# Brown-LEMS/Edge_Based_Visual_Odometry

Measured on AMD Instinct MI355X. Metric: stereo pairs/sec (TOED+NCC match) on KITTI 1241×376; achieved HBM GB/s, higher is better.
Workload: dtype f64; 1 GPU; configs[1]: single KITTI-shaped stereo pair 1241x376 (generator S2, scene 7+rank, 12 px disparity), TOED both images (fp64, no FMA, bit-exact) + epipolar/disparity/orientation candidate search + NCC, resident in HBM, replayed; toed_mode=hybrid, edges_left=126184, edges_right=126340, candidate_pairs=581657, ncc_matches=472947, sims_stored=False, pairs_in_flight_per_gpu=6, streams_per_gpu=4, pairs_submitted_as_hipgraph=2331, toed_strict_fallbacks=0, parallelism=1 independent sequence(s), one per GPU, no collective

## Files before the change

edge_based_visual_odometry_amd/csrc/match_kernels.hip:

```cpp
#include <atomic>
#include <cstdlib>

#include "ebvo_cand.h"
#include "ebvo_internal.h"
#include "ebvo_math.h"

namespace
{

constexpr int BATCH = 64;
constexpr int TILE = 64;
constexpr int STAGE = 64;
struct DevPairs
{
    int64_t host;
    const int32_t *row_ptr;
    DevN nL;
    int64_t cap;
};
__device__ inline int64_t devpairs(const DevPairs &d)
{
    const int64_t n = d.row_ptr ? (int64_t)d.row_ptr[devn(d.nL)] : d.host;
    return n < d.cap ? n : d.cap;
}

__device__ inline void lines_body(const double *__restrict__ F, const ebvo_edge *__restrict__ e, int n, double *__restrict__ lines,
                                  int vb, int vg)
{
    for (int k = vb * blockDim.x + threadIdx.x; k < n; k += vg * blockDim.x)
    {
        const double x = e[k].x, y = e[k].y;
#pragma unroll
        for (int r = 0; r < 3; ++r)
            lines[(size_t)k * 3 + r] = (F[r * 3 + 0] * x + F[r * 3 + 1] * y) + F[r * 3 + 2];
    }
}

__global__ void lines_kernel(const double *__restrict__ F, const ebvo_edge *__restrict__ e, DevN nd,
                             double *__restrict__ lines)
{
    lines_body(F, e, devn(nd), lines, blockIdx.x, gridDim.x);
}

__global__ __launch_bounds__(256) void boxes_kernel(const ebvo_edge *__restrict__ R, DevN nRd, Box *__restrict__ cb,
                                                    Box *__restrict__ gb, int32_t *__restrict__ tile_flag, int ntiles)
{
    boxes_body(R, devn(nRd), cb, gb, tile_flag, ntiles, blockIdx.x, gridDim.x);
}

__device__ inline Box region_box(const LeftCtx &l, double D, double band, int mask)
{
    const double inf = __builtin_inf();
    Box r;
    r.x0 = -inf; r.x1 = inf; r.y0 = -inf; r.y1 = inf;
    if (mask & EBVO_STAGE_DISPARITY)
    {
        r.x0 = l.lx - D; r.x1 = l.lx + D; r.y0 = l.ly - D; r.y1 = l.ly + D;
    }
    if ((mask & EBVO_STAGE_EPIPOLAR) && (mask & EBVO_STAGE_DISPARITY) && l.ah == l.ah && l.bh == l.bh && l.ch == l.ch)
    {
        const double m = 1e-9;
        if (fabs(l.bh) > m)
        {
            const double ya = -(l.ah * r.x0 + l.ch) / l.bh, yb = -(l.ah * r.x1 + l.ch) / l.bh;
            const double e = band / fabs(l.bh) + BOX_SLACK;
            r.y0 = fmax(r.y0, fmin(ya, yb) - e);
            r.y1 = fmin(r.y1, fmax(ya, yb) + e);
        }
        if (fabs(l.ah) > m)
        {
            const double xa = -(l.bh * r.y0 + l.ch) / l.ah, xb = -(l.bh * r.y1 + l.ch) / l.ah;
            const double e = band / fabs(l.ah) + BOX_SLACK;
            r.x0 = fmax(r.x0, fmin(xa, xb) - e);
            r.x1 = fmin(r.x1, fmax(xa, xb) + e);
        }
    }
    return r;
}

template <bool FILL, bool COPY = FILL>
__global__ __launch_bounds__(256) void candidates_kernel(const ebvo_edge *__restrict__ L,
                                                         const ebvo_edge *__restrict__ R,
                                                         const double *__restrict__ lines,
                                                         const Box *__restrict__ cb, const Box *__restrict__ gb,
                                                         CandParams P, int32_t *__restrict__ cnt,
                                                         const int32_t *__restrict__ row_ptr,
                                                         int32_t *__restrict__ col_idx,
                                                         unsigned long long *__restrict__ total_part)
{
    __shared__ double s_x[BATCH * CHUNK], s_y[BATCH * CHUNK], s_th[BATCH * CHUNK];
    __shared__ Box s_box[BATCH];
    __shared__ LeftCtx s_left[TILE];
    __shared__ int s_round[256];
    __shared__ int s_groups[256];
    __shared__ int s_wcnt[4];
    __shared__ double s_red[4];
    __shared__ unsigned long long s_tot[4];

    const int tid = threadIdx.x, lane = tid & 63, wid = tid >> 6;
    constexpr int LPE = CHUNK, GPB = 256 / LPE, ROUNDS = TILE / GPB;
    constexpr unsigned long long GMASK = (1ull << LPE) - 1ull;
    static_assert(TILE % GPB == 0 && BATCH % LPE == 0 && BATCH <= 64, "tile rounds / marked-chunk mask");
    const int gid = tid / LPE, e = tid % LPE, gshift = lane & ~(LPE - 1);
    const int nL = devn(P.nL), nR = devn(P.nR);
    const int nchunks = (nR + CHUNK - 1) / CHUNK, ngroups = (nchunks + GROUP - 1) / GROUP;
    const double d2 = P.max_disp * P.max_disp;
    const double D = P.max_disp + BOX_SLACK, band = P.epi_thr + BOX_SLACK;
    const double inf = __builtin_inf();
    unsigned long long blk_total = 0;

    auto compact = [&](bool sel, int value, int *list) -> int {
        const unsigned long long m = __ballot(sel);
        if (lane == 0)
            s_wcnt[wid] = __popcll(m);
        __syncthreads();
        int pre = 0, tot = 0;
#pragma unroll
        for (int k = 0; k < 4; ++k)
        {
            if (k < wid) pre += s_wcnt[k];
            tot += s_wcnt[k];
        }
        if (sel)
            list[pre + __popcll(m & ((1ull << lane) - 1ull))] = value;
        __syncthreads();
        return tot;
    };

    if (!FILL && blockIdx.x == 0 && tid == 0)
        cnt[nL] = 0;
    if (FILL && COPY)
    {
        const int e16 = tid & 15;
        const int rows = (gridDim.x * 256) >> 4;
        for (int i = (blockIdx.x * 256 + tid) >> 4; i < nL; i += rows)
        {
            const int64_t o = row_ptr[i];
            const int n = row_ptr[i + 1] - row_ptr[i];
            if (n > STAGE)
                continue;
            for (int k = e16; k < n; k += 16)
                if (o + k < P.cap)
                    col_idx[o + k] = P.stage[(size_t)i * STAGE + k];
        }
    }
    for (int tile = blockIdx.x; tile * TILE < nL; tile += gridDim.x)
    {
        if (FILL && !P.tile_flag[tile])
            continue;
        if (wid == 0)
        {
            const int i = tile * TILE + lane;
            const bool live = i < nL;
            const int il = live ? i : 0;
            const LeftCtx l = left_ctx_make(L[il].x, L[il].y, L[il].theta, lines[(size_t)il * 3], lines[(size_t)il * 3 + 1],
                                            lines[(size_t)il * 3 + 2], P.epi_thr, d2);
            Box rb = region_box(l, D, band, P.mask);
            if (!live) { rb.x0 = inf; rb.x1 = -inf; rb.y0 = inf; rb.y1 = -inf; }
            s_left[lane] = l;
            const double a0 = wave_min(rb.x0), a1 = wave_max(rb.x1), b0 = wave_min(rb.y0), b1 = wave_max(rb.y1);
            if (lane == 0) { s_red[0] = a0; s_red[1] = a1; s_red[2] = b0; s_red[3] = b1; }
        }
        __syncthreads();
        Box U;
        U.x0 = s_red[0]; U.x1 = s_red[1]; U.y0 = s_red[2]; U.y1 = s_red[3];
        auto meets_union = [&](const Box &bx) {
            return !(bx.x0 > U.x1 || bx.x1 < U.x0 || bx.y0 > U.y1 || bx.y1 < U.y0);
        };

        int n[ROUNDS];
        int64_t o[ROUNDS];
#pragma unroll
        for (int r = 0; r < ROUNDS; ++r)
        {
            n[r] = 0;
            o[r] = 0;
        }
        if (FILL)
        {
#pragma unroll
            for (int r = 0; r < ROUNDS; ++r)
            {
                const int i = tile * TILE + r * GPB + gid;
                o[r] = (int64_t)row_ptr[i < nL ? i : 0];
            }
        }
        for (int g0 = 0; g0 < ngroups; g0 += 256)
        {
            const int g = g0 + tid;
            const int ngsel = compact(g < ngroups && meets_union(gb[g < ngroups ? g : 0]), g, s_groups);
            for (int q = 0; q < ngsel; q += 4)
            {
                const int gq = q + (tid >> 6);
                const int c = (gq < ngsel) ? s_groups[gq] * GROUP + (tid & 63) : nchunks;
                const int nsel = compact(c < nchunks && meets_union(cb[c < nchunks ? c : 0]), c, s_round);
                for (int b0 = 0; b0 < nsel; b0 += BATCH)
                {
                    const int mb = min(BATCH, nsel - b0);
                    for (int idx = tid; idx < mb * CHUNK; idx += 256)
                    {
                        const int k = s_round[b0 + idx / CHUNK] * CHUNK + (idx % CHUNK);
                        double x = __builtin_nan(""), y = x, th = x;
                        if (k < nR)
                        {
                            x = R[k].x; y = R[k].y; th = R[k].theta;
                        }
                        s_x[idx] = x; s_y[idx] = y; s_th[idx] = th;
                    }
                    if (tid < mb)
                        s_box[tid] = cb[s_round[b0 + tid]];
                    __syncthreads();
#pragma unroll
                    for (int r = 0; r < ROUNDS; ++r)
                    {
                        const int li = r * GPB + gid;
                        const int i = tile * TILE + li;
                        const bool live = i < nL;
                        const LeftCtx l = s_left[li];
                        unsigned long long pm = 0;
#pragma unroll
                        for (int k = 0; k < BATCH / LPE; ++k)
                        {
                            const int j = k * LPE + e;
                            const bool may = live && j < mb &&
                                             box_may_match(s_box[j < mb ? j : 0], l.lx, l.ly, l.ah, l.bh, l.ch, D, band,
                                                           P.mask);
                            const unsigned long long bal = __ballot(may);
                            pm |= ((bal >> gshift) & GMASK) << (LPE * k);
                        }
                        while (__any(pm != 0))
                        {
                            const bool act = pm != 0;
                            const int j = act ? __ffsll((long long)pm) - 1 : 0;
                            pm &= pm - 1;
                            const int idx = j * CHUNK + e;
                            const bool ok = act && pair_passes(l, s_x[idx], s_y[idx], s_th[idx], P);
                            const unsigned hits = (unsigned)((__ballot(ok) >> gshift) & GMASK);
                            if (ok)
                            {
                                const int rank = __popc(hits & ((1u << e) - 1u));
                                const int k = s_round[b0 + j] * CHUNK + e;
                                if (FILL)
                                {
                                    if (o[r] + rank < P.cap)
                                        col_idx[o[r] + rank] = k;
                                }
                                else if (n[r] + rank < STAGE)
                                    P.stage[(size_t)i * STAGE + n[r] + rank] = k;
                            }
                            const int nh = __popc(hits);
                            n[r] += nh;
                            o[r] += nh;
                        }
                    }
                    __syncthreads();
                }
            }
        }
        if (!FILL)
        {
            unsigned long long tsum = 0;
#pragma unroll
            for (int r = 0; r < ROUNDS; ++r)
            {
                const int i = tile * TILE + r * GPB + gid;
                if (e == 0 && i < nL)
                {
                    cnt[i] = n[r];
                    if (n[r] > STAGE)
                        P.tile_flag[tile] = 1;
                    tsum += (unsigned long long)n[r];
                }
            }
            for (int d = 32; d > 0; d >>= 1)
                tsum += __shfl_down(tsum, d);
            if (lane == 0)
                s_tot[wid] = tsum;
            __syncthreads();
            if (tid == 0)
            {
                const unsigned long long t = s_tot[0] + s_tot[1] + s_tot[2] + s_tot[3];
                blk_total += t;
                P.tile_tot[tile] = (int32_t)(uint32_t)t;
            }
        }
        __syncthreads();
    }
    if (!FILL && tid == 0)
        total_part[blockIdx.x] = blk_total;
}

__global__ void total_sum_kernel(const unsigned long long *__restrict__ part, int n, unsigned long long *__restrict__ total)
{
    unsigned long long v = 0;
    for (int k = threadIdx.x; k < n; k += 64)
        v += part[k];
    for (int d = 32; d > 0; d >>= 1)
        v += __shfl_down(v, d);
    if (threadIdx.x == 0)
        *total = v;
}

__global__ void candidates_copy_kernel(const int32_t *__restrict__ row_ptr, const int32_t *__restrict__ stage, DevN nLd,
                                       int64_t cap, int32_t *__restrict__ col_idx)
{
    const int nL = devn(nLd);
    const int e = threadIdx.x & 15;
    const int rows = (gridDim.x * blockDim.x) >> 4;
    for (int i = (blockIdx.x * blockDim.x + threadIdx.x) >> 4; i < nL; i += rows)
    {
        const int64_t o = row_ptr[i];
        const int n = row_ptr[i + 1] - row_ptr[i];
        if (n > STAGE)
            continue;
        for (int k = e; k < n; k += 16)
            if (o + k < cap)
                col_idx[o + k] = stage[(size_t)i * STAGE + k];
    }
}

struct ClearList
{
    int32_t *p[EBVO_CLEAR_MAX];
    int n[EBVO_CLEAR_MAX];
};
__global__ void clear_kernel(ClearList C)
{
    int32_t *__restrict__ p = C.p[blockIdx.y];
    const int n = C.n[blockIdx.y];
    for (int k = blockIdx.x * blockDim.x + threadIdx.x; k < n; k += gridDim.x * blockDim.x)
        p[k] = 0;
}

constexpr int SCAN_ITEMS = 16;
constexpr int SCAN_BLOCK = 256;
constexpr int SCAN_TILE = SCAN_ITEMS * SCAN_BLOCK;
constexpr int SCAN_BATCH = 4;
constexpr int SCAN_DIRECT_TILES = 16;

struct ScanBatch
{
    const int32_t *in[SCAN_BATCH];
    int32_t *out[SCAN_BATCH];
    DevN n[SCAN_BATCH];
    int n_add;
    int32_t *total[SCAN_BATCH];
    int32_t *sums;
    int tiles;
    int direct;
};

__device__ inline int32_t block_sum_256(int32_t v, int32_t *wsum)
{
    for (int d = 32; d > 0; d >>= 1)
        v += __shfl_down(v, d);
    if ((threadIdx.x & 63) == 0)
        wsum[threadIdx.x >> 6] = v;
    __syncthreads();
    return wsum[0] + wsum[1] + wsum[2] + wsum[3];
}

__global__ __launch_bounds__(SCAN_BLOCK) void scan_reduce_kernel(ScanBatch S)
{
    __shared__ int32_t wsum[SCAN_BLOCK / 64];
    const int a = blockIdx.y;
    const int n_in = devn(S.n[a]), n = n_in + S.n_add;
    const int base = blockIdx.x * SCAN_TILE;
    if (base >= n)
        return;
    const int32_t *__restrict__ in = S.in[a];
    int32_t v = 0;
#pragma unroll
    for (int t = 0; t < SCAN_ITEMS; ++t)
    {
        const int k = base + t * SCAN_BLOCK + threadIdx.x;
        v += (k < n_in) ? in[k] : 0;
    }
    const int32_t tot = block_sum_256(v, wsum);
    if (threadIdx.x == 0)
        S.sums[(size_t)a * S.tiles + blockIdx.x] = tot;
}

__global__ __launch_bounds__(SCAN_BLOCK) void scan_apply_kernel(ScanBatch S)
{
    __shared__ int32_t wsum[SCAN_BLOCK / 64], wpre[SCAN_BLOCK / 64];
    const int a = blockIdx.y;
    const int n_in = devn(S.n[a]), n = n_in + S.n_add;
    const int base = blockIdx.x * SCAN_TILE + threadIdx.x * SCAN_ITEMS;
    if (blockIdx.x * SCAN_TILE >= n)
        return;
    const int32_t *__restrict__ in = S.in[a];
    int32_t *__restrict__ out = S.out[a];
    int32_t o = 0;
    if (S.direct)
    {
        const int before = min((int)blockIdx.x * SCAN_TILE, n_in);
        if ((reinterpret_cast<uintptr_t>(in) & 15) == 0)
        {
            const int4 *p4 = reinterpret_cast<const int4 *>(in);
            for (int k = threadIdx.x; k < (before >> 2); k += SCAN_BLOCK)
            {
                const int4 q = p4[k];
                o += (q.x + q.y) + (q.z + q.w);
            }
            for (int k = (before & ~3) + threadIdx.x; k < before; k += SCAN_BLOCK)
                o += in[k];
        }
        else
            for (int k = threadIdx.x; k < before; k += SCAN_BLOCK)
                o += in[k];
    }
    else
        for (int k = threadIdx.x; k < (int)blockIdx.x; k += SCAN_BLOCK)
            o += S.sums[(size_t)a * S.tiles + k];
    const int32_t tile_off = block_sum_256(o, wpre);
    int32_t v[SCAN_ITEMS];
    int32_t s = 0;
    if (base + SCAN_ITEMS <= n_in && (reinterpret_cast<uintptr_t>(in + base) & 15) == 0)
    {
        const int4 *p = reinterpret_cast<const int4 *>(in + base);
#pragma unroll
        for (int t = 0; t < SCAN_ITEMS / 4; ++t)
        {
            const int4 q = p[t];
            v[4 * t] = q.x; v[4 * t + 1] = q.y; v[4 * t + 2] = q.z; v[4 * t + 3] = q.w;
        }
    }
    else
    {
#pragma unroll
        for (int t = 0; t < SCAN_ITEMS; ++t)
            v[t] = (base + t < n_in) ? in[base + t] : 0;
    }
#pragma unroll
    for (int t = 0; t < SCAN_ITEMS; ++t)
        s += v[t];
    const int lane = threadIdx.x & 63, wid = threadIdx.x >> 6;
    int32_t incl = s;
    for (int d = 1; d < 64; d <<= 1)
    {
        const int32_t t = __shfl_up(incl, d);
        if (lane >= d)
            incl += t;
    }
    if (lane == 63)
        wsum[wid] = incl;
    __syncthreads();
    int32_t pre = 0;
#pragma unroll
    for (int k = 0; k < SCAN_BLOCK / 64; ++k)
        if (k < wid)
            pre += wsum[k];
    int32_t run = tile_off + pre + incl - s;
#pragma unroll
    for (int t = 0; t < SCAN_ITEMS; ++t)
    {
        if (base + t < n)
            out[base + t] = run;
        if (S.n_add == 1 && base + t == n_in && S.total[a])
            *S.total[a] = run;
        run += v[t];
    }
}

__global__ void gather_edges_kernel(const ebvo_edge *__restrict__ R, const int32_t *__restrict__ idx, int64_t n,
                                    ebvo_edge *__restrict__ out)
{
    const int64_t k = (int64_t)blockIdx.x * blockDim.x + threadIdx.x;
    if (k < n)
        out[k] = R[idx[k]];
}

__device__ inline double bilinear_nan(const uint8_t *__restrict__ img, int rows, int cols, int pitch, double x,
                                      double y)
{
    const double x1 = floor(x), x2 = ceil(x);
    const double yc = ceil(y), yf = floor(y);
    const bool inside = (x1 >= 0) && (yf >= 0) && (x2 < cols) && (yc < rows);
    const int c1 = inside ? (int)x1 : 0;
    const int r1 = inside ? (int)yc * pitch : 0, r2 = inside ? (int)yf * pitch : 0;
    unsigned short p1, p2;
    __builtin_memcpy(&p1, img + r1 + c1, 2);
    __builtin_memcpy(&p2, img + r2 + c1, 2);
    const double I11 = (double)(p1 & 0xff);
    const double I21 = (double)(p1 >> 8);
    const double I12 = (double)(p2 & 0xff);
    const double I22 = (double)(p2 >> 8);
    const double wxa = x2 - x;
    const double wxb = x - x1;
    const double wya = -(yf - y);
    const double wyb = -(y - yc);
    const double f1 = wxa * I11 + wxb * I21;
    const double f2 = wxa * I12 + wxb * I22;
    const double v = wya * f1 + wyb * f2;
    const bool ok = inside && (x2 != x1) && (yf != yc);
    return ok ? v : __builtin_nan("");
}

template <int CTRL>
__device__ inline double dpp_f64(double v)
{
    const int lo = __double2loint(v), hi = __double2hiint(v);
    const int plo = __builtin_amdgcn_update_dpp(0, lo, CTRL, 0xf, 0xf, true);
    const int phi = __builtin_amdgcn_update_dpp(0, hi, CTRL, 0xf, 0xf, true);
    return __hiloint2double(phi, plo);
}

__device__ inline double butterfly8(double s)
{
    s += dpp_f64<0xB1>(s);
    s += dpp_f64<0x4E>(s);
    s += dpp_f64<0x141>(s);
    return s;
}

struct PatchBatch
{
    const uint8_t *img[2];
    const ebvo_edge *edges[2];
    DevN n[2];
    double2 *sc[2];
    float *raw[2], *norm[2];
    uint8_t *flag[2];
};

__device__ inline void sincos_body(const ebvo_edge *__restrict__ e, int n, double2 *__restrict__ sc, int vb, int vg)
{
    for (int k = vb * blockDim.x + threadIdx.x; k < n; k += vg * blockDim.x)
    {
        double sn, cs;
        ebvo_sincos(e[k].theta, &sn, &cs);
        double2 v;
// ... 1666 lines not shown
```

Measured before the change: 3524 stereo pairs/s.

## Use precomputed region-box overlap test for flat epipolar bands in candidate search

For each left edge, the region box and a flag saying whether its epipolar band is nearly axis-aligned are now stored in shared memory. For flagged edges, the per-chunk box_may_match test is replaced by a cheaper four-compare overlap ballot against that stored box. Other edges use an inlined box test built on raw v_min/v_max f64 instructions. The change also stages boxes for all batch slots and masks the result with a staged-bit mask, and sets launch_bounds to 4 blocks per CU. The overlap test on flat regions is looser than the epipolar test, so more chunks may reach pair_passes, and the inline-asm min/max drops NaN handling.

```diff
diff --git a/edge_based_visual_odometry_amd/csrc/match_kernels.hip b/edge_based_visual_odometry_amd/csrc/match_kernels.hip
--- a/edge_based_visual_odometry_amd/csrc/match_kernels.hip
+++ b/edge_based_visual_odometry_amd/csrc/match_kernels.hip
@@ -48,6 +48,31 @@
     boxes_body(R, devn(nRd), cb, gb, tile_flag, ntiles, blockIdx.x, gridDim.x);
 }
 
+__device__ inline double fmin_q(double a, double b)
+{
+    double r;
+    asm("v_min_f64 %0, %1, %2" : "=v"(r) : "v"(a), "v"(b));
+    return r;
+}
+__device__ inline double fmax_q(double a, double b)
+{
+    double r;
+    asm("v_max_f64 %0, %1, %2" : "=v"(r) : "v"(a), "v"(b));
+    return r;
+}
+__device__ inline double wave_min_q(double v)
+{
+    for (int d = 32; d > 0; d >>= 1)
+        v = fmin_q(v, __shfl_xor(v, d));
+    return v;
+}
+__device__ inline double wave_max_q(double v)
+{
+    for (int d = 32; d > 0; d >>= 1)
+        v = fmax_q(v, __shfl_xor(v, d));
+    return v;
+}
+
 __device__ inline Box region_box(const LeftCtx &l, double D, double band, int mask)
 {
     const double inf = __builtin_inf();
@@ -64,22 +89,59 @@
         {
             const double ya = -(l.ah * r.x0 + l.ch) / l.bh, yb = -(l.ah * r.x1 + l.ch) / l.bh;
             const double e = band / fabs(l.bh) + BOX_SLACK;
-            r.y0 = fmax(r.y0, fmin(ya, yb) - e);
-            r.y1 = fmin(r.y1, fmax(ya, yb) + e);
+            r.y0 = fmax_q(r.y0, fmin_q(ya, yb) - e);
+            r.y1 = fmin_q(r.y1, fmax_q(ya, yb) + e);
         }
         if (fabs(l.ah) > m)
         {
             const double xa = -(l.bh * r.y0 + l.ch) / l.ah, xb = -(l.bh * r.y1 + l.ch) / l.ah;
             const double e = band / fabs(l.ah) + BOX_SLACK;
-            r.x0 = fmax(r.x0, fmin(xa, xb) - e);
-            r.x1 = fmin(r.x1, fmax(xa, xb) + e);
+            r.x0 = fmax_q(r.x0, fmin_q(xa, xb) - e);
+            r.x1 = fmin_q(r.x1, fmax_q(xa, xb) + e);
         }
     }
     return r;
 }
 
+__device__ inline bool box_may_match_q(const Box &bx, double xl, double yl, double ah, double bh, double ch, double D,
+                                       double band, int mask)
+{
+    double x0 = bx.x0, x1 = bx.x1, y0 = bx.y0, y1 = bx.y1;
+    bool out = false;
+    if (mask & EBVO_STAGE_DISPARITY)
+    {
+        x0 = fmax_q(x0, xl - D);
+        x1 = fmin_q(x1, xl + D);
+        y0 = fmax_q(y0, yl - D);
+        y1 = fmin_q(y1, yl + D);
+        out = x0 > x1 || y0 > y1;
+    }
+    if (mask & EBVO_STAGE_EPIPOLAR)
+    {
+        const double gx0 = ah * x0, gx1 = ah * x1, gy0 = bh * y0, gy1 = bh * y1;
+        const double gmin = fmin_q(gx0, gx1) + fmin_q(gy0, gy1) + ch;
+        const double gmax = fmax_q(gx0, gx1) + fmax_q(gy0, gy1) + ch;
+        out = out || gmin > band || gmax < -band;
+    }
+    return !out;
+}
+
+__device__ inline unsigned long long region_ballot(const Box bx, const Box r)
+{
+    constexpr int UGE = 11, ULE = 13;
+    return __builtin_amdgcn_fcmp(bx.x0, r.x1, ULE) & __builtin_amdgcn_fcmp(bx.x1, r.x0, UGE) &
+           __builtin_amdgcn_fcmp(bx.y0, r.y1, ULE) & __builtin_amdgcn_fcmp(bx.y1, r.y0, UGE);
+}
+
+constexpr double FLAT_BANDS = 4.0;
+__device__ inline bool region_is_flat(const LeftCtx &l, double D, double band)
+{
+    const double p = fabs(l.ah), q = fabs(l.bh);
+    return 2.0 * D * fmin(p, q) <= FLAT_BANDS * band * fmax(p, q);
+}
+
 template <bool FILL, bool COPY = FILL>
-__global__ __launch_bounds__(256) void candidates_kernel(const ebvo_edge *__restrict__ L,
+__global__ __launch_bounds__(256, 4) void candidates_kernel(const ebvo_edge *__restrict__ L,
                                                          const ebvo_edge *__restrict__ R,
                                                          const double *__restrict__ lines,
                                                          const Box *__restrict__ cb, const Box *__restrict__ gb,
@@ -91,6 +153,8 @@
     __shared__ double s_x[BATCH * CHUNK], s_y[BATCH * CHUNK], s_th[BATCH * CHUNK];
     __shared__ Box s_box[BATCH];
     __shared__ LeftCtx s_left[TILE];
+    __shared__ Box s_region[TILE];
+    __shared__ int s_flat[TILE];
     __shared__ int s_round[256];
     __shared__ int s_groups[256];
     __shared__ int s_wcnt[4];
@@ -107,6 +171,7 @@
     const double d2 = P.max_disp * P.max_disp;
     const double D = P.max_disp + BOX_SLACK, band = P.epi_thr + BOX_SLACK;
     const double inf = __builtin_inf();
+    const bool both_stages = (P.mask & EBVO_STAGE_EPIPOLAR) && (P.mask & EBVO_STAGE_DISPARITY);
     unsigned long long blk_total = 0;
 
     auto compact = [&](bool sel, int value, int *list) -> int {
@@ -158,7 +223,9 @@
             Box rb = region_box(l, D, band, P.mask);
             if (!live) { rb.x0 = inf; rb.x1 = -inf; rb.y0 = inf; rb.y1 = -inf; }
             s_left[lane] = l;
-            const double a0 = wave_min(rb.x0), a1 = wave_max(rb.x1), b0 = wave_min(rb.y0), b1 = wave_max(rb.y1);
+            s_region[lane] = rb;
+            s_flat[lane] = both_stages && region_is_flat(l, D, band);
+            const double a0 = wave_min_q(rb.x0), a1 = wave_max_q(rb.x1), b0 = wave_min_q(rb.y0), b1 = wave_max_q(rb.y1);
             if (lane == 0) { s_red[0] = a0; s_red[1] = a1; s_red[2] = b0; s_red[3] = b1; }
         }
         __syncthreads();
@@ -207,8 +274,9 @@
                         }
                         s_x[idx] = x; s_y[idx] = y; s_th[idx] = th;
                     }
-                    if (tid < mb)
-                        s_box[tid] = cb[s_round[b0 + tid]];
+                    if (tid < BATCH)
+                        s_box[tid] = cb[tid < mb ? s_round[b0 + tid] : 0];
+                    const unsigned long long staged = mb < 64 ? (1ull << mb) - 1ull : ~0ull;
                     __syncthreads();
 #pragma unroll
                     for (int r = 0; r < ROUNDS; ++r)
@@ -218,16 +286,28 @@
                         const bool live = i < nL;
                         const LeftCtx l = s_left[li];
                         unsigned long long pm = 0;
-#pragma unroll
-                        for (int k = 0; k < BATCH / LPE; ++k)
+                        if (live && s_flat[li])
                         {
-                            const int j = k * LPE + e;
-                            const bool may = live && j < mb &&
-                                             box_may_match(s_box[j < mb ? j : 0], l.lx, l.ly, l.ah, l.bh, l.ch, D, band,
-                                                           P.mask);
-                            const unsigned long long bal = __ballot(may);
-                            pm |= ((bal >> gshift) & GMASK) << (LPE * k);
+                            const Box rg = s_region[li];
+#pragma unroll
+                            for (int k = 0; k < BATCH / LPE; ++k)
+                            {
+                                const Box bx = s_box[k * LPE + e];
+                                pm |= ((region_ballot(bx, rg) >> gshift) & GMASK) << (LPE * k);
+                            }
                         }
+                        else if (live)
+                        {
+                            const double ah = s_left[li].ah, bh = s_left[li].bh, ch = s_left[li].ch;
+#pragma unroll 2
+                            for (int k = 0; k < BATCH / LPE; ++k)
+                            {
+                                const Box bx = s_box[k * LPE + e];
+                                const unsigned long long bal = __ballot(box_may_match_q(bx, l.lx, l.ly, ah, bh, ch, D, band, P.mask));
+                                pm |= ((bal >> gshift) & GMASK) << (LPE * k);
+                            }
+                        }
+                        pm &= staged;
                         while (__any(pm != 0))
                         {
                             const bool act = pm != 0;
```

New measurement: 3569 stereo pairs/s, median of 6. +1.3%, better.
